# jczarnowski/DeepFactors

Hardware: NVIDIA H100
Metric: keyframe-pair Jacobian+JtJ evals/sec (640x480, C=32) (higher is better)
Workload: dtype f32

## Files before the change

### deepfactors_b200/_lib.py

```python
from __future__ import annotations

import ctypes as C
import os

_HERE = os.path.dirname(os.path.abspath(__file__))
LIB_PATH = os.environ.get("DFK_LIB") or os.path.join(_HERE, "libdfk.so")

DFK_OK = 0
DFK_ERR_INVALID_ARG = 1
DFK_ERR_CUDA = 2
DFK_ERR_UNSUPPORTED = 3
DFK_ERR_NOMEM = 4

DFK_GRAM_AUTO, DFK_GRAM_FP32, DFK_GRAM_TF32X3 = 0, 1, 2


class DfkError(RuntimeError):

    def __init__(self, status: int, message: str):
        super().__init__(f"dfk status {status}: {message}")
        self.status = status
        self.message = message


# ... 173 lines not shown


class DfkBowQuery(C.Structure):
    _fields_ = [("vector", DfkBowVector), ("max_results", C.c_int32), ("max_id", C.c_int32)]


class DfkBowScoreItem(C.Structure):
    _fields_ = [("entry", C.c_int32), ("vector", DfkBowVector)]


BOW_TRAIN_MAX_ROUNDS = 1000
BOW_TRAIN_MAX_DESCRIPTORS = 268435456


class DfkBowTrainDesc(C.Structure):
    _fields_ = [("k", C.c_int32), ("L", C.c_int32), ("descriptor_bytes", C.c_int32), ("num_images", C.c_int32),
                ("seed", C.c_uint64), ("num_descriptors", C.c_int64), ("descriptors_dev", C.c_void_p),
                ("image_offsets", C.c_void_p)]


class DfkBowTrainStats(C.Structure):
    _fields_ = [("num_nodes", C.c_int32), ("num_words", C.c_int32), ("max_rounds", C.c_int32),
                ("capped_nodes", C.c_int32), ("empty_clusters", C.c_int32),
                ("level_max_rounds", C.c_int32 * BOW_MAX_DEPTH)]


class DfkBowVocabularyShape(C.Structure):
    _fields_ = [("k", C.c_int32), ("L", C.c_int32), ("weighting", C.c_int32), ("scoring", C.c_int32),
                ("descriptor_bytes", C.c_int32), ("num_nodes", C.c_int32), ("num_words", C.c_int32)]


WINDOW_ERROR_DOUBLES = 7
WINDOW_ERROR_EX_DOUBLES = 8


_F = C.POINTER(C.c_float)
_IMG = C.POINTER(DfkImage)
_CAM = C.POINTER(DfkCamera)
_H = C.c_void_p
SYMBOLS = {
    "dfk_create": (C.c_int, [C.c_int, C.POINTER(_H)]),
    "dfk_destroy": (C.c_int, [_H]),
    "dfk_set_stream": (C.c_int, [_H, C.c_void_p]),
    "dfk_set_sm_limit": (C.c_int, [_H, C.c_int]),
    "dfk_use_own_stream": (C.c_int, [_H]),
    "dfk_get_stream": (C.c_void_p, [_H]),
    "dfk_synchronize": (C.c_int, [_H]),
    "dfk_last_error": (C.c_char_p, [_H]),
    "dfk_status_string": (C.c_char_p, [C.c_int]),
    "dfk_version": (C.c_int, []),
    "dfk_sfm_supports_code_size": (C.c_int, [C.c_int]),
    "dfk_set_profiling": (C.c_int, [_H, C.c_int]),
    "dfk_get_profile": (C.c_int, [_H, C.POINTER(C.c_double), C.POINTER(C.c_uint64), C.POINTER(C.c_uint64)]),
    "dfk_sfm_set_params": (C.c_int, [_H, C.POINTER(DfkSfmAlignerParams)]),
    "dfk_sfm_get_params": (C.c_int, [_H, C.POINTER(DfkSfmAlignerParams)]),
    "dfk_sfm_set_gram_mode": (C.c_int, [_H, C.c_int]),
    "dfk_se3_set_huber_delta": (C.c_int, [_H, C.c_float]),
    "dfk_sfm_run_step": (C.c_int, [_H, _F, _F, _F, C.c_int, _CAM, _IMG, _IMG, _IMG, _IMG, _IMG, _IMG, _IMG,
                                   _F, _F, _F, C.POINTER(C.c_uint64)]),
    "dfk_sfm_evaluate_error": (C.c_int, [_H, _F, _F, _CAM, _IMG, _IMG, _IMG, _IMG, _IMG, _F,
                                         C.POINTER(C.c_uint64)]),
    "dfk_sfm_evaluate_error_batch": (C.c_int, [_H, C.POINTER(DfkSfmWorkItem), C.c_int, C.c_void_p]),
    "dfk_sfm_run_step_batch": (C.c_int, [_H, C.POINTER(DfkSfmWorkItem), C.c_int, C.c_int, C.c_void_p]),
    "dfk_sfm_run_step_batch_host": (C.c_int, [_H, C.POINTER(DfkSfmWorkItem), C.c_int, C.c_int, _F]),
    "dfk_sfm_stream_create": (C.c_int, [_H, C.c_int, C.c_int, C.c_size_t, C.c_int, C.POINTER(C.c_void_p)]),
    "dfk_sfm_stream_destroy": (C.c_int, [_H, C.c_void_p]),
    "dfk_sfm_stream_submit": (C.c_int, [_H, C.c_void_p, C.POINTER(DfkSfmWorkItem), C.c_int, C.POINTER(C.c_uint64)]),
    "dfk_sfm_stream_wait": (C.c_int, [_H, C.c_void_p, C.c_uint64, _F]),
    "dfk_window_create": (C.c_int, [_H, C.POINTER(DfkWindowDesc), C.POINTER(C.c_void_p)]),
    "dfk_window_destroy": (C.c_int, [_H, C.c_void_p]),
    "dfk_window_floats": (C.c_size_t, [C.c_void_p]),
    "dfk_window_assemble": (C.c_int, [_H, C.c_void_p, C.c_void_p, C.c_void_p]),
    "dfk_window_create_geometric": (C.c_int, [_H, C.POINTER(DfkWindowDesc), C.c_int, C.POINTER(C.c_int32),
                                              C.POINTER(C.c_int32), C.POINTER(C.c_void_p)]),
    "dfk_window_assemble_geometric": (C.c_int, [_H, C.c_void_p, C.c_void_p, C.c_void_p, C.c_void_p]),
    "dfk_window_create_frames": (C.c_int, [_H, C.POINTER(DfkWindowDesc), C.c_int, C.POINTER(C.c_int32),
                                           C.POINTER(C.c_int32), C.c_int, C.POINTER(C.c_void_p)]),
    "dfk_window_marginalize_frames": (C.c_int, [_H, C.c_void_p, C.c_void_p, C.c_int, C.POINTER(C.c_int32), C.c_void_p,
                                                C.c_void_p]),
    "dfk_window_add_priors": (C.c_int, [_H, C.c_void_p, C.c_int, C.POINTER(C.c_int32), C.c_void_p, C.c_void_p,
                                        C.c_void_p]),
    "dfk_window_create_priors": (C.c_int, [_H, C.POINTER(DfkWindowDesc), C.c_int, C.POINTER(C.c_int32),
                                           C.POINTER(C.c_int32), C.c_int, C.c_int, C.POINTER(C.c_int32),
                                           C.POINTER(C.c_int32), C.POINTER(C.c_void_p)]),
    "dfk_window_add_keyframe_priors": (C.c_int, [_H, C.c_void_p, C.c_void_p, C.c_void_p, C.c_void_p]),
    "dfk_window_blanket": (C.c_int, [_H, C.c_void_p, C.c_int, C.POINTER(C.c_int32), C.POINTER(C.c_int32)]),
    "dfk_window_marginalize_keyframe": (C.c_int, [_H, C.c_void_p, C.c_void_p, C.c_void_p, C.c_int, C.c_int, C.c_void_p,
                                                  C.c_void_p, C.c_void_p, C.c_void_p, C.c_double,
                                                  C.POINTER(C.c_double), C.c_void_p, C.c_void_p]),
    "dfk_window_solver_create": (C.c_int, [_H, C.c_void_p, C.c_int, C.POINTER(C.c_int32), C.POINTER(C.c_void_p)]),
    "dfk_window_solver_destroy": (C.c_int, [_H, C.c_void_p]),
    "dfk_window_solver_tiles": (C.c_int, [_H, C.c_void_p, C.POINTER(C.c_size_t)]),
    "dfk_window_solve": (C.c_int, [_H, C.c_void_p, C.c_void_p, C.POINTER(DfkWindowSolveParams), C.POINTER(C.c_double),
                                   C.c_void_p, C.c_void_p]),
    "dfk_window_solver_update": (C.c_int, [_H, C.c_void_p, C.c_void_p, C.POINTER(DfkWindowUpdateParams),
                                           C.POINTER(C.c_double), C.c_void_p, C.c_void_p, C.POINTER(C.c_int32)]),
    "dfk_window_solver_create_from": (C.c_int, [_H, C.c_void_p, C.c_int, C.POINTER(C.c_int32), C.c_void_p,
                                                C.POINTER(C.c_void_p)]),
    "dfk_window_problem_create": (C.c_int, [_H, C.POINTER(DfkWindowProblemDesc), C.POINTER(C.c_void_p)]),
    "dfk_window_problem_destroy": (C.c_int, [_H, C.c_void_p]),
    "dfk_window_problem_set_state": (C.c_int, [_H, C.c_void_p, C.c_void_p, C.c_void_p]),
    "dfk_window_problem_get_state": (C.c_int, [_H, C.c_void_p, C.c_void_p, C.c_void_p]),
    "dfk_window_problem_linearize": (C.c_int, [_H, C.c_void_p, C.c_void_p]),
    "dfk_window_problem_error": (C.c_int, [_H, C.c_void_p, C.c_void_p]),
    "dfk_window_problem_retract": (C.c_int, [_H, C.c_void_p, C.c_void_p]),
    "dfk_window_problem_error_ex": (C.c_int, [_H, C.c_void_p, C.c_void_p]),
# ... 112 lines not shown
```

### deepfactors_b200/csrc/dfk_api.cu

```cuda
#include <cuda_runtime.h>
#include <math.h>
#include <stdint.h>
#include <stdio.h>
#include <stdlib.h>
#include <string.h>

#include <algorithm>
#include <cmath>
#include <memory>
#include <new>
#include <string>
#include <vector>

#include "dfk.h"
#include "dfk_host.h"
#include "dfk_internal.h"
#include "dfk_se3.cuh"

using namespace dfk;

struct DfkSfmStream {
  int device = 0, code_size = 0, max_items = 0, depth = 0;
  size_t max_bytes = 0;
  cudaStream_t copy_stream = nullptr;
// ... 259 lines not shown
namespace {

DfkStatus cache_ray_tables(DfkHandle h, SfmItemDev* items, int n)
{
  h->ray_pending.clear();
  if (h->ray_flush) {
    h->ray_cache.clear();
    h->ray_flush = false;
  }
  for (int i = 0; i < n; ++i) {
    SfmItemDev& d = items[i];
    const uint32_t W = d.width, H = d.height;
    size_t rt = 0;
    for (const auto& r : h->ray_cache) {
      if (r.fx == d.fx && r.fy == d.fy && r.u0 == d.u0 && r.v0 == d.v0 && r.w == W && r.h == H) break;
      ++rt;
    }
    if (rt == h->ray_cache.size()) {
      if (rt >= 256) h->ray_flush = true;
      DfkContext::RayTab r{d.fx, d.fy, d.u0, d.v0, W, H, {}, false};
      if (r.dev.ensure((size_t)W + H) != cudaSuccess)
        return fail(h, DFK_ERR_CUDA, "[SfmAligner::RunStep] scratch allocation failed");
      h->ray_cache.push_back(std::move(r));
    }
    d.ray_tab = h->ray_cache[rt].dev.ptr;
    if (!h->ray_cache[rt].built) h->ray_pending.push_back(rt);
  }
  return DFK_OK;
}

DfkStatus run_batch(DfkHandle h, const DfkSfmWorkItem* items, int n, int code_size, float* records_dev)
{
  if (!items || n <= 0 || !records_dev) return fail(h, DFK_ERR_INVALID_ARG, "[SfmAligner::RunStep] null/empty batch");
  StepKernel k;
  DFK_TRY(choose_step_kernel(h, items, n, code_size, &k));
  DeviceGuard guard(h->device);
  SfmLaunchPlan plan;
  bool any_fused = false;
  for (int i = 0; i < n; ++i) any_fused = any_fused || items[i].code != nullptr;
  if (any_fused)
    DFK_CUDA(h, h->codes_dev.ensure((size_t)n * code_size), "[SfmAligner::RunStep] scratch allocation failed");
  h->items_host.resize(n);
  DFK_TRY(build_items(h, items, n, code_size, k.tile_px, k.max_ctas, h->codes_dev.ptr, h->items_host.data(), &plan));
  DFK_TRY(cache_ray_tables(h, h->items_host.data(), n));
  if (any_fused) {
    h->codes_host.assign((size_t)n * code_size, 0.0f);
    for (int i = 0; i < n; ++i)
      if (items[i].code)
        memcpy(h->codes_host.data() + (size_t)i * code_size, items[i].code, sizeof(float) * code_size);
    DFK_CUDA(h, cudaMemcpyAsync(h->codes_dev.ptr, h->codes_host.data(), sizeof(float) * (size_t)n * code_size,
                                cudaMemcpyHostToDevice, h->stream),
             "[SfmAligner::RunStep] code upload failed");
  }
  DFK_CUDA(h, h->items_dev.ensure((size_t)n), "[SfmAligner::RunStep] scratch allocation failed");
  DFK_CUDA(h, h->partials_dev.ensure((size_t)plan.num_partials * k.pfloats), "[SfmAligner::RunStep] scratch allocation failed");
  SfmItemDev* items_dev = h->items_dev.ptr;
  DFK_CUDA(h, cudaMemcpyAsync(items_dev, h->items_host.data(), sizeof(SfmItemDev) * n, cudaMemcpyHostToDevice, h->stream),
           "[SfmAligner::RunStep] work list upload failed");
  if (!h->ray_pending.empty()) {
    DFK_CUDA(h, launch_sfm_ray_tables(items_dev, n, h->stream), "[SfmAligner::RunStep] kernel launch failed");
    for (size_t rt : h->ray_pending) h->ray_cache[rt].built = true;
    h->launches += 1;
  }
  return launch_step(h, k, code_size, items_dev, n, plan, h->partials_dev.ptr, records_dev);
}

}

extern "C" {

int dfk_version(void) { return DFK_VERSION; }

const char* dfk_status_string(DfkStatus s)
{
  switch (s) {
    case DFK_OK: return "ok";
    case DFK_ERR_INVALID_ARG: return "invalid argument";
    case DFK_ERR_CUDA: return "CUDA error";
    case DFK_ERR_UNSUPPORTED: return "unsupported";
    case DFK_ERR_NOMEM: return "out of memory";
  }
  return "unknown";
}

int dfk_sfm_supports_code_size(int code_size)
{
  return (sfm_fp32_supported(code_size) || sfm_wide_supported(code_size)) ? 1 : 0;
}

DfkStatus dfk_create(int device, DfkHandle* out)
{
  try {
    if (!out) return DFK_ERR_INVALID_ARG;
    *out = nullptr;
    int count = 0;
    cudaError_t e = cudaGetDeviceCount(&count);
    if (e != cudaSuccess || count == 0) return DFK_ERR_CUDA;
    if (device < 0) {
      if (cudaGetDevice(&device) != cudaSuccess) return DFK_ERR_CUDA;
    }
    if (device >= count) return DFK_ERR_INVALID_ARG;
    DfkContext* h = new (std::nothrow) DfkContext();
    if (!h) return DFK_ERR_NOMEM;
    h->device = device;
    h->params.sfmparams = DfkDenseSfmParams{0.1f, 1000.f, 2.0f, 0.0f, 2};
    h->params.step_threads = 32; h->params.step_blocks = 11; h->params.eval_threads = 224; h->params.eval_blocks = 66;
    DeviceGuard guard(device);
    bool ok = true;
    ok = ok && cudaDeviceGetAttribute(&h->num_sms, cudaDevAttrMultiProcessorCount, device) == cudaSuccess;
    ok = ok && cudaStreamCreateWithFlags(&h->own_stream, cudaStreamNonBlocking) == cudaSuccess;
    h->stream = h->own_stream;
// ... 31 lines not shown
  });
}

DfkStatus dfk_use_own_stream(DfkHandle h)
{
  return guarded(h, [&] {
    h->stream = h->own_stream;
    return DFK_OK;
  });
}

DfkStatus dfk_set_sm_limit(DfkHandle h, int num_sms)
{
  return guarded(h, [&] {
    if (num_sms < 0) return fail(h, DFK_ERR_INVALID_ARG, "[dfk_set_sm_limit] num_sms < 0");
    h->sm_limit = num_sms;
    return DFK_OK;
  });
}

void* dfk_get_stream(DfkHandle h) { return h ? h->stream : nullptr; }

DfkStatus dfk_synchronize(DfkHandle h)
{
  return guarded(h, [&] {
    DeviceGuard guard(h->device);
    DFK_CUDA(h, cudaStreamSynchronize(h->stream), "stream synchronize failed");
    return DFK_OK;
  });
}

const char* dfk_last_error(DfkHandle h) { return h ? h->err.c_str() : "null handle"; }

DfkStatus dfk_set_profiling(DfkHandle h, int enabled)
{
  return guarded(h, [&] {
    h->profiling = enabled != 0;
    return DFK_OK;
  });
}

DfkStatus dfk_get_profile(DfkHandle h, double* main_kernel_ms, uint64_t* main_kernel_launches,
                          uint64_t* total_kernel_launches)
{
  return guarded(h, [&] {
    DeviceGuard guard(h->device);
    DFK_TRY(drain_events(h));
    if (main_kernel_ms) *main_kernel_ms = h->ev_ms_accum;
    if (main_kernel_launches) *main_kernel_launches = h->ev_count_accum;
    if (total_kernel_launches) *total_kernel_launches = h->launches;
    h->ev_ms_accum = 0.0;
    h->ev_count_accum = 0;
    h->launches = 0;
    return DFK_OK;
  });
}

DfkStatus dfk_sfm_set_params(DfkHandle h, const DfkSfmAlignerParams* p)
{
  return guarded(h, [&] {
    if (!p) return DFK_ERR_INVALID_ARG;
    if (p->step_threads % 32 != 0 || p->eval_threads % 32 != 0)
      return fail(h, DFK_ERR_INVALID_ARG, "threads must be a multiple of 32!");
    if (p->step_blocks > 1024 || p->eval_blocks > 1024) return fail(h, DFK_ERR_INVALID_ARG, "blocks must be less than 1024");
    if (p->sfmparams.valid_border < 1)
      return fail(h, DFK_ERR_INVALID_ARG, "valid_border must be >= 1 (bilinear sampling reads ix+1, iy+1)");
    h->params = *p;
    return DFK_OK;
  });
}

DfkStatus dfk_sfm_get_params(DfkHandle h, DfkSfmAlignerParams* p)
{
  return guarded(h, [&] {
    if (!p) return DFK_ERR_INVALID_ARG;
    *p = h->params;
    return DFK_OK;
  });
}

DfkStatus dfk_sfm_set_gram_mode(DfkHandle h, DfkGramMode m)
{
  return guarded(h, [&] {
    if (m != DFK_GRAM_AUTO && m != DFK_GRAM_FP32 && m != DFK_GRAM_TF32X3)
      return fail(h, DFK_ERR_INVALID_ARG, "unknown gram mode");
    h->gram_mode = m;
    return DFK_OK;
  });
}

DfkStatus dfk_se3_set_huber_delta(DfkHandle h, float v)
{
  return guarded(h, [&] {
    h->se3_huber_delta = v;
    return DFK_OK;
  });
}

DfkStatus dfk_sfm_run_step_batch(DfkHandle h, const DfkSfmWorkItem* items, int n, int code_size, float* records_dev)
{
  return guarded(h, [&] { return run_batch(h, items, n, code_size, records_dev); });
}

DfkStatus dfk_sfm_run_step_batch_host(DfkHandle h, const DfkSfmWorkItem* items, int n, int code_size,
                                      float* records_host)
{
// ... 853 lines not shown
```

### deepfactors_b200/csrc/dfk_host.h

```cpp
#pragma once

#include <cuda_runtime.h>
#include <stdint.h>
#include <string.h>

#include <algorithm>
#include <string>
#include <vector>

#include "dfk.h"
#include "dfk_internal.h"
#include "dfk_se3.cuh"

using namespace dfk;

template <typename T, bool Pinned>
struct Scratch {
  T* ptr = nullptr;
  size_t cap = 0;

  Scratch() = default;
  Scratch(Scratch&& o) noexcept : ptr(o.ptr), cap(o.cap) { o.ptr = nullptr; o.cap = 0; }
  ~Scratch() { release(); }

// ... 35 lines not shown

  DeviceBuf<float> simple_scratch;
  DeviceBuf<unsigned int> counter;
  DeviceBuf<float> out_dev;
  PinnedBuf<float> out_host;
  DeviceBuf<float> code_dev;
  std::vector<unsigned char> staging;
  DeviceBuf<unsigned char> batch_dev;
  PinnedBuf<unsigned char> batch_host;
  DeviceBuf<float> batch_partials;
  DeviceBuf<unsigned int> batch_counters;
  DeviceBuf<unsigned char> eval_descs;
  DeviceBuf<float> eval_partials;
  DeviceBuf<unsigned int> eval_counters;
  DeviceBuf<unsigned char> depth_dev;
  DeviceBuf<unsigned char> depth_prior_dev;
  DeviceBuf<float> depth_prior_partials;

  DeviceBuf<unsigned char> sparse_dev;
  PinnedBuf<unsigned char> sparse_host;
  DeviceBuf<unsigned char> rep_dev;
  DeviceBuf<unsigned char> geo_dev;
  DeviceBuf<SfmItemDev> items_dev;
  DeviceBuf<float> partials_dev;
  DeviceBuf<unsigned char> match_items;
  DeviceBuf<unsigned char> match_scratch;
  DeviceBuf<unsigned char> orb_items;
  DeviceBuf<unsigned char> orb_scratch;
  DeviceBuf<unsigned char> orb_pyr_dev;
  DeviceBuf<unsigned char> pp_dev;
  DeviceBuf<double> pp_partials;
  DeviceBuf<unsigned char> mesh_dev;
  DeviceBuf<unsigned char> mesh_scratch;
  DeviceBuf<unsigned char> bow_dev;
  DeviceBuf<int32_t> bow_words;
  DeviceBuf<unsigned char> bow_scratch;
  DeviceBuf<int> window_lists;
  DeviceBuf<unsigned char> marg_lists;
  DeviceBuf<unsigned char> marg_dev;
  struct RayTab {
    float fx, fy, u0, v0;
    uint32_t w, h;
    DeviceBuf<float> dev;
    bool built;
  };
  std::vector<RayTab> ray_cache;
  std::vector<size_t> ray_pending;
  bool ray_flush = false;
  DeviceBuf<float> codes_dev;
  std::vector<float> codes_host;
  DeviceBuf<float> records_dev;
  PinnedBuf<float> records_host;
  std::vector<SfmItemDev> items_host;

  bool profiling = false;
  std::vector<cudaEvent_t> ev_pool;
  size_t ev_used = 0;
  double ev_ms_accum = 0.0;
  uint64_t ev_count_accum = 0;
  uint64_t launches = 0;

  ~DfkContext()
  {
    for (cudaEvent_t e : ev_pool) cudaEventDestroy(e);
    if (own_stream) cudaStreamDestroy(own_stream);
  }
};

inline DfkStatus fail(DfkHandle h, DfkStatus s, const std::string& msg)
{
  if (h) h->err = msg;
  return s;
}

inline DfkStatus oom(DfkHandle h) noexcept
{
  if (h) {
    try {
      h->err = "out of host memory";
    } catch (...) {
    }
  }
  return DFK_ERR_NOMEM;
}

template <class F>
DfkStatus guarded(DfkHandle h, F&& body) noexcept
{
  if (!h) return DFK_ERR_INVALID_ARG;
  try {
    return body();
  } catch (...) {
    return oom(h);
  }
}

inline DfkStatus cuda_fail(DfkHandle h, cudaError_t e, const char* what)
{
  std::string m = std::string(what) + ": " + cudaGetErrorString(e);
  cudaGetLastError();
  return fail(h, DFK_ERR_CUDA, m);
}

#define DFK_CUDA(h, call, what)                            \
  do {                                                     \
    cudaError_t e__ = (call);                              \
// ... 305 lines not shown
```

### deepfactors_b200/csrc/dfk_internal.h

```cpp
#pragma once

#include <cuda_runtime.h>
#include <stdint.h>

#include <string>
#include <vector>

#include "dfk.h"
#include "dfk_preprocess_model.h"

namespace dfk {

template <class T>
struct Part {
  size_t off = 0;
  T* at(void* base) const { return reinterpret_cast<T*>(static_cast<unsigned char*>(base) + off); }
};

struct Layout {
  size_t bytes = 0;
  template <class T>
  Part<T> add(size_t count)
  {
    const Part<T> p{bytes};
// ... 22 lines not shown
  uint32_t num_pixels;
  uint32_t tile_begin;
  uint32_t num_tiles;
  uint32_t perm_mul;
  uint32_t mag_tiles;
  uint32_t mag_width;
  uint32_t first_cta, num_ctas, partial_begin;
  uint32_t flags;
  float* dpt_out;
  uint32_t dpt_out_pitch;
  const float* code;
  const float* ray_tab;
  float P0[36];
  float P1[36];
};

enum : uint32_t { ITEM_FLAG_BULK = 1u, ITEM_FLAG_GRAD_ALIGNED = 2u, ITEM_FLAG_FUSED_DEPTH = 4u };

template <int C>
struct SfmCfg {
  static constexpr int NF = C + 7;
  static constexpr int NFP = (NF + 7) & ~7;
  static constexpr int NB = NFP / 8;
  static constexpr int NBLK = NB * (NB + 1) / 2;
  static constexpr int PARTIAL_FLOATS = NFP * NFP + 8;
};

constexpr int kTilePixels = 256;

template <int C>
struct TcCfg {
  static constexpr int S = C - 8;
  static constexpr int F = C + 8;
  static constexpr int ROWS = 2 * C;
  static constexpr int COLS = C + 24;
  static constexpr int PARTIAL_FLOATS = ROWS * COLS + 8;
  static constexpr int INLIERS = ROWS * COLS;
  __host__ __device__ static constexpr int hh(int i, int j) { return j * ROWS + S + i; }
  __host__ __device__ static constexpr int lh(int i, int j) { return i < S ? j * ROWS + i : (16 + i) * ROWS + S + j; }
};

constexpr int kSfmTcTilePixels = 128;
constexpr int sfm_tc_ctas_per_sm(int code_size) { return code_size <= 32 ? 4 : (code_size <= 64 ? 2 : 1); }
__host__ __device__ constexpr bool sfm_tc_writes_d(int code_size) { return code_size > 32; }
constexpr size_t sfm_tc_partial_floats(int code_size) { return (size_t)(2 * code_size) * (code_size + 24) + 8; }

struct SfmLaunchPlan {
  int num_items = 0;
  int num_tiles = 0;
  int num_ctas = 0;
  int num_partials = 0;
};

cudaError_t launch_sfm_fp32(int code_size, const SfmItemDev* items_dev, const SfmLaunchPlan& plan,
                            float* partials_dev, cudaStream_t stream, cudaEvent_t ev_start = nullptr,
                            cudaEvent_t ev_stop = nullptr);
cudaError_t launch_sfm_ray_tables(const SfmItemDev* items_dev, int num_items, cudaStream_t stream);
cudaError_t launch_sfm_finalize(int code_size, bool tc, const SfmItemDev* items_dev, int num_items,
                                const float* partials_dev, float* records_dev, cudaStream_t stream);
constexpr int sfm_wide_tile_pixels(int code_size) { return code_size >= 128 ? 64 : 128; }
bool sfm_wide_supported(int code_size);
cudaError_t launch_sfm_wide(int code_size, const SfmItemDev* items_dev, const SfmLaunchPlan& plan,
                            float* partials_dev, cudaStream_t stream, cudaEvent_t ev_start = nullptr,
                            cudaEvent_t ev_stop = nullptr);
bool sfm_tc_supported(int code_size);
cudaError_t launch_sfm_tc(int code_size, const SfmItemDev* items_dev, const SfmLaunchPlan& plan, float* partials_dev,
                          cudaStream_t stream, cudaEvent_t ev_start = nullptr, cudaEvent_t ev_stop = nullptr);
size_t sfm_partial_floats(int code_size);
constexpr int sfm_fp32_ctas_per_sm(int code_size) { return code_size <= 8 ? 2 : 1; }
bool sfm_fp32_supported(int code_size);
int sfm_max_ctas();

struct PixelCam {
  float q[4], t[3];
  float fx, fy, u0, v0, border, ulim, vlim, min_dpt;
};
struct View {
  const float* ptr;
  uint32_t pitch;
};
int grid_for(int area);
struct Se3TrackDesc {
  PixelCam pc;
  View img0, img1, dpt0, grad1;
  int width, height;
  int nblocks;
  int grad_aligned;
};
cudaError_t launch_se3_step(const Se3TrackDesc& d, float huber_delta, float* scratch, unsigned int* counter, float* out,
                            float* pose, float* history, cudaStream_t s);
cudaError_t launch_se3_step(const Se3TrackDesc* descs_dev, int num_problems, int max_blocks, float huber_delta,
                            float* scratch, int scratch_stride, unsigned int* counters, float* outs, float* poses,
                            cudaStream_t s);
struct EvalErrorDesc {
  PixelCam pc;
  View img0, img1, dpt0;
  int width, height;
  int nblocks;
  int scratch_row;
};
cudaError_t launch_eval_error(const EvalErrorDesc& d, float huber_delta, float* scratch, unsigned int* counter,
                              float* out, cudaStream_t s);
cudaError_t launch_eval_error(const EvalErrorDesc* descs_dev, int num_items, int max_blocks, float huber_delta,
                              float* scratch, unsigned int* counters, float* outs, cudaStream_t s);
struct DepthDecodeDesc {
  View prx, jac;
// ... 450 lines not shown
```

### deepfactors_b200/csrc/dfk_sfm_finalize.cu

```cuda
#include <cuda_runtime.h>
#include <stdint.h>

#include "dfk_internal.h"

namespace dfk {

namespace {

constexpr int kFinWarps = 8;
constexpr int kFinUnroll = 4;

__device__ __forceinline__ int packed_index(int i, int j, int NP) { return i * NP - (i * (i - 1)) / 2 + (j - i); }

template <int C, bool TC>
__global__ void __launch_bounds__(kFinWarps * 32)
sfm_finalize_kernel(const SfmItemDev* __restrict__ items, const float* __restrict__ partials,
                    float* __restrict__ records)
{
  using Cfg = SfmCfg<C>;
  constexpr int NFP = Cfg::NFP;
  constexpr int NP = 12 + C;
  constexpr int NH = NP * (NP + 1) / 2;
  constexpr int REC = NH + NP + 2;
  constexpr int NE = (C + 7 > 49) ? (C + 7) : 49;
  constexpr int EPL = (NE + 31) / 32;
  using Tc = TcCfg<C>;
  constexpr int PSTRIDE = TC ? Tc::PARTIAL_FLOATS : Cfg::PARTIAL_FLOATS;
  constexpr int INL_OFF = TC ? Tc::INLIERS : NFP * NFP;
  constexpr int NOFF = TC ? 3 : 1;
  __shared__ float red[kFinWarps][EPL * 32];
  __shared__ unsigned int red_inl[kFinWarps];
  __shared__ float sum[EPL * 32];

  cudaGridDependencySynchronize();
  const SfmItemDev& I = items[blockIdx.x];
  const int unit = blockIdx.y;
  const int warp = threadIdx.x >> 5, lane = threadIdx.x & 31;
  const float* P = partials + (size_t)I.partial_begin * PSTRIDE;
  const int np = (int)I.num_ctas;

  int off[EPL][NOFF];
  bool act[EPL];
#pragma unroll
  for (int q = 0; q < EPL; ++q) {
    const int e = q * 32 + lane;
    int fi, fj;
    if (unit < C) {
      act[q] = (unit + e) < (C + 7);
      fi = unit;
      fj = unit + e;
    } else {
      const int r = e / 7, c = e - 7 * r;
      act[q] = (e < 49) && (c >= r);
      fi = C + r;
      fj = C + c;
    }
    if (!act[q]) {
      fi = 0;
      fj = 0;
    }
    if constexpr (TC) {
      off[q][0] = Tc::hh(fi, fj);
      off[q][1] = Tc::lh(fi, fj);
      off[q][2] = Tc::lh(fj, fi);
    } else {
      off[q][0] = fi * NFP + fj;
    }
  }
  float part[EPL];
#pragma unroll
  for (int q = 0; q < EPL; ++q) part[q] = 0.0f;
  unsigned int inl = 0;
  for (int k0 = warp; k0 < np; k0 += kFinWarps * kFinUnroll) {
    float v[kFinUnroll][EPL];
    unsigned int vi[kFinUnroll];
#pragma unroll
    for (int u = 0; u < kFinUnroll; ++u) {
      const int k = k0 + u * kFinWarps;
      const bool on = k < np;
      const float* Pk = P + (size_t)(on ? k : 0) * PSTRIDE;
#pragma unroll
      for (int q = 0; q < EPL; ++q) {
        v[u][q] = 0.0f;
        if (on && act[q]) {
          if constexpr (TC) v[u][q] = (Pk[off[q][0]] + Pk[off[q][1]]) + Pk[off[q][2]];
          else v[u][q] = Pk[off[q][0]];
        }
// ... 127 lines not shown
```

### deepfactors_b200/csrc/dfk_sfm_tc.cu

```cuda
#include <cuda_runtime.h>
#include <stdint.h>

#include "dfk_async.cuh"
#include "dfk_geom.cuh"
#include "dfk_internal.h"
#include "dfk_sfm_frontend.cuh"
#include "dfk_wgmma.cuh"

namespace dfk {

namespace {

constexpr int TILE = kSfmTcTilePixels;
constexpr uint32_t kLbo = 128 + 16;
constexpr uint32_t kSbo = 32 * kLbo + 16;
#ifndef DFK_FLUSH_TILES
#define DFK_FLUSH_TILES 8
#endif
constexpr int kFlushTiles = DFK_FLUSH_TILES;

template <int C>
struct WgCfg {
  using T = TcCfg<C>;
  static constexpr int NWG = C >= 128 ? 2 : 1;
// ... 280 lines not shown
    if constexpr (W::NWG > 1) __syncthreads();
#pragma unroll
    for (int i4 = 0; i4 < NQ; ++i4) {
      if (i4 >= PRE) load_quad(i4);
      const float sk = __shfl_sync(0xffffffffu, feat[0], 4 * i4 + r);
#pragma unroll
      for (int cb = 0; cb < NCB; ++cb) {
        const float x[4] = {sk * v[i4][cb].x, sk * v[i4][cb].y, sk * v[i4][cb].z, sk * v[i4][cb].w};
        const uint32_t gh = code_h + (uint32_t)(4 * cb) * kSbo;
        const uint32_t gl = cb < NCB - 1 ? code_l + (uint32_t)(4 * cb) * kSbo : code_l_last;
#pragma unroll
        for (int e = 0; e < 4; ++e) {
          const float h = tf32_trunc(x[e]);
          const uint32_t off = (uint32_t)i4 * kLbo + (uint32_t)e * 16u;
          sts32(gh + off, h);
          sts32(gl + off, x[e] - h);
        }
      }
    }
    if (lane < PW) {
#pragma unroll
      for (int f = 0; f < 7; ++f) {
        const float h = tf32_trunc(feat[1 + f]);
        sts32(pose_h + (uint32_t)f * 16u, h);
        sts32(pose_l + (uint32_t)f * 16u, feat[1 + f] - h);
      }
    }
    fence_proxy_async_smem();
    const int nv = __syncthreads_count(ok);
    if (nv > 0) {
      wgmma_fence();
#pragma unroll
      for (int kk = 0; kk < TILE / 8; ++kk) {
        const uint32_t k_off = (uint32_t)kk * 2u * kLbo;
        const bool accumulate = kk > 0 || chain_valid > 0;
#ifndef DFK_EXP_NOMMA
        const uint64_t b_desc = make_wgmma_desc_kmajor(op + (uint32_t)W::G_H * kSbo + k_off, kLbo, kSbo);
#pragma unroll
        for (int t = 0; t < MT; ++t)
          wgmma_tf32<N>(acc[t], make_wgmma_desc_kmajor(op + (uint32_t)(8 * (MT * wg + t)) * kSbo + k_off, kLbo, kSbo),
                        b_desc, accumulate);
#endif
      }
      wgmma_commit();
    }
    chain_valid += nv;
    inliers += (unsigned)nv;
    ++tiles_in_chain;
#ifdef DFK_EXP_CTA_CLOCKS
    valid_tiles += nv > 0;
#endif
  }
  flush(true);
#ifdef DFK_EXP_CTA_CLOCKS
  __syncthreads();
  if (tid == 0 && blockIdx.x < kClockCtas) {
    unsigned int smid;
    asm volatile("mov.u32 %0, %%smid;" : "=r"(smid));
    unsigned long long* o = g_cta_clocks[blockIdx.x];
    o[0] = t_entry;
    o[1] = global_ns();
    o[2] = ((unsigned long long)ntiles << 32) | (unsigned)valid_tiles;
    o[3] = smid;
  }
#endif
}

template <int C>
cudaError_t launch_impl(const SfmItemDev* items_dev, const SfmLaunchPlan& plan, float* partials_dev,
                        cudaStream_t stream, cudaEvent_t ev_start, cudaEvent_t ev_stop)
{
  constexpr size_t smem = sizeof(Smem<C>);
  if constexpr (smem > 48 * 1024) {
    const cudaError_t err =
        cudaFuncSetAttribute(sfm_step_tc_kernel<C>, cudaFuncAttributeMaxDynamicSharedMemorySize, (int)smem);
    if (err != cudaSuccess) return err;
  }
  if (ev_start) cudaEventRecord(ev_start, stream);
  sfm_step_tc_kernel<C><<<plan.num_ctas, WgCfg<C>::THREADS, smem, stream>>>(items_dev, plan.num_tiles, partials_dev);
  if (ev_stop) cudaEventRecord(ev_stop, stream);
  return cudaGetLastError();
}

}

bool sfm_tc_supported(int code_size) { return code_size == 32 || code_size == 64 || code_size == 128; }

cudaError_t launch_sfm_tc(int code_size, const SfmItemDev* items_dev, const SfmLaunchPlan& plan, float* partials_dev,
                          cudaStream_t stream, cudaEvent_t ev_start, cudaEvent_t ev_stop)
{
  switch (code_size) {
    case 32: return launch_impl<32>(items_dev, plan, partials_dev, stream, ev_start, ev_stop);
    case 64: return launch_impl<64>(items_dev, plan, partials_dev, stream, ev_start, ev_stop);
    case 128: return launch_impl<128>(items_dev, plan, partials_dev, stream, ev_start, ev_stop);
    default: return cudaErrorInvalidValue;
  }
}

}

#ifdef DFK_EXP_CTA_CLOCKS
extern "C" int dfk_exp_cta_clocks(unsigned long long* out, int n)
{
  if (n < 0 || n > dfk::kClockCtas) return -1;
  if (cudaDeviceSynchronize() != cudaSuccess) return -1;
  return cudaMemcpyFromSymbol(out, dfk::g_cta_clocks, sizeof(unsigned long long) * 4 * (size_t)n) == cudaSuccess ? 0 : -1;
// ... 3 lines not shown
```

### deepfactors_b200/csrc/dfk_window.cu

```cuda
#include <cuda_runtime.h>
#include <stdint.h>

#include "dfk_internal.h"

namespace dfk {

namespace {

__device__ __forceinline__ int packed_index(int i, int j, int NP) { return i * NP - (i * (i - 1)) / 2 + (j - i); }
__device__ __forceinline__ float rec_h(const float* rec, int a, int b, int NP)
{
  return a <= b ? rec[packed_index(a, b, NP)] : rec[packed_index(b, a, NP)];
}

__device__ __forceinline__ int link_row0(int r) { return r < 6 ? r : 6 + r; }
__device__ __forceinline__ int link_row1(int r, int C) { return r < 6 ? 6 + r : 6 + C + r; }

__global__ void __launch_bounds__(256)
window_assemble_kernel(WindowDev w, const float* __restrict__ records, const float* __restrict__ geo,
                       float* __restrict__ out)
{
  const int C = w.code_size, B = 6 + C, NP = 12 + C;
  const int NH = NP * (NP + 1) / 2, REC = NH + NP + 2;
  const int NG = 12 + 2 * C, NHG = NG * (NG + 1) / 2, RECG = NHG + NG + 2;
  float* tail = out + (size_t)w.num_keyframes * (B * B + B) + (size_t)w.num_pairs * B * 6;
  const int job = blockIdx.x;
  if (job < w.num_keyframes) {
    const int k = job;
    float* D = out + (size_t)k * B * B;
    float* g = out + (size_t)w.num_keyframes * B * B + (size_t)k * B;
    const int a0 = w.kf0_ptr[k], a1 = w.kf0_ptr[k + 1];
    const int b0 = w.kf1_ptr[k], b1 = w.kf1_ptr[k + 1];
    const int l00 = w.lk0_ptr[k], l01 = w.lk0_ptr[k + 1];
    const int l10 = w.lk1_ptr[k], l11 = w.lk1_ptr[k + 1];
    for (int e = threadIdx.x; e < B * B + B; e += blockDim.x) {
      float s = 0.0f;
      if (e < B * B) {
        const int r = e / B, c = e - r * B;
        const int lr = r < 6 ? r : 6 + r, lc = c < 6 ? c : 6 + c;
        for (int q = a0; q < a1; ++q) s += rec_h(records + (size_t)w.kf0_items[q] * REC, lr, lc, NP);
        if (r < 6 && c < 6)
          for (int q = b0; q < b1; ++q) s += rec_h(records + (size_t)w.kf1_items[q] * REC, 6 + r, 6 + c, NP);
        for (int q = l00; q < l01; ++q) s += rec_h(geo + (size_t)w.lk0_links[q] * RECG, link_row0(r), link_row0(c), NG);
        for (int q = l10; q < l11; ++q)
          s += rec_h(geo + (size_t)w.lk1_links[q] * RECG, link_row1(r, C), link_row1(c, C), NG);
        D[e] = s;
      } else {
        const int r = e - B * B;
        const int lr = r < 6 ? r : 6 + r;
        for (int q = a0; q < a1; ++q) s -= records[(size_t)w.kf0_items[q] * REC + NH + lr];
        if (r < 6)
          for (int q = b0; q < b1; ++q) s -= records[(size_t)w.kf1_items[q] * REC + NH + 6 + r];
        for (int q = l00; q < l01; ++q) s -= geo[(size_t)w.lk0_links[q] * RECG + NHG + link_row0(r)];
        for (int q = l10; q < l11; ++q) s -= geo[(size_t)w.lk1_links[q] * RECG + NHG + link_row1(r, C)];
        g[r] = s;
      }
    }
  } else if (job < w.num_keyframes + w.num_pairs) {
    const int p = job - w.num_keyframes;
    float* O = out + (size_t)w.num_keyframes * (B * B + B) + (size_t)p * B * 6;
    const int i0 = w.pair_ptr[p], i1 = w.pair_ptr[p + 1];
    for (int e = threadIdx.x; e < B * 6; e += blockDim.x) {
      const int r = e / 6, c = e - r * 6;
      const int lr = r < 6 ? r : 6 + r;
      float s = 0.0f;
      for (int q = i0; q < i1; ++q) s += rec_h(records + (size_t)w.pair_items[q] * REC, lr, 6 + c, NP);
      O[e] = s;
    }
  } else if (job < w.num_keyframes + w.num_pairs + w.num_links) {
    const int l = job - w.num_keyframes - w.num_pairs;
    float* O = tail + 2 + (size_t)l * B * B;
    const float* rec = geo + (size_t)l * RECG;
    for (int e = threadIdx.x; e < B * B; e += blockDim.x) {
      const int r = e / B, c = e - r * B;
      O[e] = rec_h(rec, link_row0(r), link_row1(c, C), NG);
    }
  } else if (job < w.num_keyframes + w.num_pairs + w.num_links + w.num_frames) {
    const int f = job - w.num_keyframes - w.num_pairs - w.num_links;
    float* Df = tail + 2 + (size_t)w.num_links * B * B + (size_t)f * 36;
    float* gf = tail + 2 + (size_t)w.num_links * B * B + (size_t)w.num_frames * 36 + (size_t)f * 6;
    const int p = w.frame_pair[f];
    const int i0 = w.pair_ptr[p], i1 = w.pair_ptr[p + 1];
    for (int e = threadIdx.x; e < 42; e += blockDim.x) {
      float s = 0.0f;
      if (e < 36) {
        const int r = e / 6, c = e - r * 6;
        for (int q = i0; q < i1; ++q) s += rec_h(records + (size_t)w.pair_items[q] * REC, 6 + r, 6 + c, NP);
        Df[e] = s;
// ... 394 lines not shown
      for (int r = threadIdx.x; r < nB; r += blockDim.x) {
        double Gd = 0.0;
        for (int c = 0; c < nB; ++c) Gd = __fma_rn(P[(size_t)r * nB + c], d[c], Gd);
        gd = __fma_rn(P[(size_t)nB * nB + r], d[r], gd);
        dGd = __fma_rn(d[r], Gd, dGd);
      }
      gd = block_sum(gd, red);
      dGd = block_sum(dGd, red);
      f = __dadd_rn(f, __dadd_rn(__fma_rn(-2.0, gd, P[(size_t)nB * nB + nB]), dGd));
    }
  }
  if (threadIdx.x == 0) {
    if (md.w > 0.0) {
      double cc = 0.0;
      for (int c = 0; c < C; ++c) cc = __fma_rn(md.code[c], md.code[c], cc);
      f = __fma_rn(md.w, cc, f);
    }
    *md.f = f;
    *md.info = 0;
  }
}

__global__ void __launch_bounds__(256)
window_marg_finalize_kernel(int C, KfMargDev md, int num_tiles, double* __restrict__ prior)
{
  const int B = 6 + C, n = md.n, nB = n * B;
  const bool bad = *md.info != 0;
  const int u = blockIdx.x, nt = n * (n + 1) / 2;
  if (u < nt) {
    const int t = n + 1 + u, I = md.tile_row[t], J = md.tile_col[t];
    const double* T = md.tiles + (size_t)t * B * B;
    for (int e = threadIdx.x; e < B * B; e += blockDim.x) {
      const int r = e / B, c = e - r * B;
      if (I == J && r < c) continue;
      const double v = bad ? 0.0 : T[e];
      prior[(size_t)((I - 1) * B + r) * nB + (J - 1) * B + c] = v;
      prior[(size_t)((J - 1) * B + c) * nB + (I - 1) * B + r] = v;
    }
    return;
  }
  for (int v = threadIdx.x; v < nB; v += blockDim.x) prior[(size_t)nB * nB + v] = bad ? 0.0 : md.rhs[B + v];
  if (threadIdx.x == 0) {
    double zz = 0.0;
    for (int r = 0; r < B; ++r) zz = __fma_rn(md.rhs[r], md.rhs[r], zz);
    prior[(size_t)nB * nB + nB] = bad ? 0.0 : __dsub_rn(*md.f, zz);
  }
}

}

cudaError_t launch_window_assemble(const WindowDev& w, const float* records_dev, const float* geo_records_dev,
                                   float* out_dev, cudaStream_t stream)
{
  window_assemble_kernel<<<w.num_keyframes + w.num_pairs + w.num_links + w.num_frames + 1, 256, 0, stream>>>(
      w, records_dev, geo_records_dev, out_dev);
  return cudaGetLastError();
}

cudaError_t launch_window_marginalize_frames(const WindowDev& w, const float* records_dev, int n, const int* frames_dev,
                                             double* priors_dev, int32_t* info_dev, cudaStream_t stream)
{
  window_marginalize_kernel<<<n, 256, 0, stream>>>(w, records_dev, frames_dev, priors_dev, info_dev);
  return cudaGetLastError();
}

cudaError_t launch_window_add_priors(const WindowDev& w, int m, const int* kf_ptr_dev, const int* kf_priors_dev,
                                     const double* priors_dev, const double* delta_dev, float* window_dev,
                                     cudaStream_t stream)
{
  window_add_priors_kernel<<<w.num_keyframes + 1, 256, 0, stream>>>(w, m, kf_ptr_dev, kf_priors_dev, priors_dev,
                                                                    delta_dev, window_dev);
  return cudaGetLastError();
}

cudaError_t launch_window_add_keyframe_priors(const WindowDev& w, const KfPriorDev& kp, const double* priors_dev,
                                              const double* delta_dev, float* window_dev, cudaStream_t stream)
{
  window_add_kf_priors_kernel<<<w.num_keyframes + kp.num_blocks + 1, 256, 0, stream>>>(w, kp, priors_dev, delta_dev,
                                                                                       window_dev);
  return cudaGetLastError();
}

cudaError_t launch_window_marg_gather(const WindowDev& w, const KfPriorDev& kp, const KfMargDev& md, int num_tiles,
                                      cudaStream_t stream)
{
  window_marg_gather_kernel<<<num_tiles + 1, 256, 0, stream>>>(w, kp, md, num_tiles);
  return cudaGetLastError();
}

cudaError_t launch_window_marg_finalize(int code_size, const KfMargDev& md, int num_tiles, double* prior_dev,
                                       cudaStream_t stream)
{
  window_marg_finalize_kernel<<<md.n * (md.n + 1) / 2 + 1, 256, 0, stream>>>(code_size, md, num_tiles, prior_dev);
  return cudaGetLastError();
}

}
```

### include/dfk.h

```cpp
#ifndef DFK_H_
#define DFK_H_

#include <stddef.h>
#include <stdint.h>

#ifdef __cplusplus
extern "C" {
#endif

#define DFK_VERSION 104

typedef enum {
  DFK_OK = 0,
  DFK_ERR_INVALID_ARG = 1,
  DFK_ERR_CUDA = 2,
  DFK_ERR_UNSUPPORTED = 3,
  DFK_ERR_NOMEM = 4
} DfkStatus;

typedef struct DfkContext* DfkHandle;

typedef struct {
  void* ptr;
  size_t pitch_bytes;
  uint32_t width;
  uint32_t height;
} DfkImage;

typedef struct {
  float fx, fy, u0, v0;
  float width, height;
} DfkCamera;

typedef struct {
  float huber_delta;
  float ocl_th;
  float avg_dpt;
  float min_dpt;
  int32_t valid_border;
} DfkDenseSfmParams;

typedef struct {
  DfkDenseSfmParams sfmparams;
  int32_t step_threads;
  int32_t step_blocks;
  int32_t eval_threads;
  int32_t eval_blocks;
} DfkSfmAlignerParams;

typedef enum { DFK_GRAM_AUTO = 0, DFK_GRAM_FP32 = 1, DFK_GRAM_TF32X3 = 2 } DfkGramMode;


DfkStatus dfk_create(int device, DfkHandle* out);
DfkStatus dfk_destroy(DfkHandle h);
DfkStatus dfk_set_stream(DfkHandle h, void* cuda_stream);
DfkStatus dfk_use_own_stream(DfkHandle h);
DfkStatus dfk_set_sm_limit(DfkHandle h, int num_sms);
void* dfk_get_stream(DfkHandle h);
DfkStatus dfk_synchronize(DfkHandle h);
const char* dfk_last_error(DfkHandle h);
const char* dfk_status_string(DfkStatus s);
int dfk_version(void);
int dfk_sfm_supports_code_size(int code_size);

DfkStatus dfk_set_profiling(DfkHandle h, int enabled);
DfkStatus dfk_get_profile(DfkHandle h, double* main_kernel_ms, uint64_t* main_kernel_launches,
                          uint64_t* total_kernel_launches);

DfkStatus dfk_sfm_set_params(DfkHandle h, const DfkSfmAlignerParams* p);
DfkStatus dfk_sfm_get_params(DfkHandle h, DfkSfmAlignerParams* p);
DfkStatus dfk_sfm_set_gram_mode(DfkHandle h, DfkGramMode m);
DfkStatus dfk_se3_set_huber_delta(DfkHandle h, float v);


DfkStatus dfk_sfm_run_step(DfkHandle h, const float pose0[7], const float pose1[7],
                           const float* code0, int code_size, const DfkCamera* cam,
                           const DfkImage* img0, const DfkImage* img1, const DfkImage* dpt0,
                           const DfkImage* std0, const DfkImage* valid0, const DfkImage* prx0_jac,
                           const DfkImage* grad1,
                           float* JtJ, float* Jtr, float* residual, uint64_t* inliers);

DfkStatus dfk_sfm_evaluate_error(DfkHandle h, const float pose0[7], const float pose1[7],
                                 const DfkCamera* cam, const DfkImage* img0, const DfkImage* img1,
                                 const DfkImage* dpt0, const DfkImage* std0, const DfkImage* grad1,
                                 float* residual, uint64_t* inliers);

typedef struct {
  float pose0[7];
  float pose1[7];
  DfkCamera cam;
  DfkImage img0, img1, dpt0, valid0, prx0_jac, grad1;
  DfkImage prx_orig;
  const float* code;
} DfkSfmWorkItem;

#define DFK_SFM_NP(C) (12 + (C))
#define DFK_SFM_RECORD_FLOATS(C) (DFK_SFM_NP(C) * (DFK_SFM_NP(C) + 1) / 2 + DFK_SFM_NP(C) + 2)

DfkStatus dfk_sfm_run_step_batch(DfkHandle h, const DfkSfmWorkItem* items, int n, int code_size,
                                 float* records_dev);
DfkStatus dfk_sfm_run_step_batch_host(DfkHandle h, const DfkSfmWorkItem* items, int n, int code_size,
                                      float* records_host);

DfkStatus dfk_sfm_evaluate_error_batch(DfkHandle h, const DfkSfmWorkItem* items, int n, float* out_dev);

typedef struct DfkSfmStream DfkSfmStream;
DfkStatus dfk_sfm_stream_create(DfkHandle h, int code_size, int max_items, size_t max_bytes_per_submit, int depth,
                                DfkSfmStream** out);
DfkStatus dfk_sfm_stream_destroy(DfkHandle h, DfkSfmStream* s);
DfkStatus dfk_sfm_stream_submit(DfkHandle h, DfkSfmStream* s, const DfkSfmWorkItem* host_items, int n,
                                uint64_t* ticket);
DfkStatus dfk_sfm_stream_wait(DfkHandle h, DfkSfmStream* s, uint64_t ticket, float* records_host);

typedef struct DfkWindow DfkWindow;
typedef struct {
  int32_t num_keyframes;
  int32_t num_pairs;
  int32_t num_items;
  int32_t code_size;
  const int32_t* pair_k0;
// ... 450 lines not shown
```

Before: 33530.

## Skip redundant work-list uploads, chain step kernels with PDL, split window assembly

Caches the last uploaded SfM work list on the host and skips the host-to-device copy when it matches byte-for-byte on the same stream. It also adds programmatic launch-completion triggers to the step and finalize kernels and launches window assembly with programmatic stream serialization, so dependent kernels can start their prologue early. The keyframe assembly job is split across several blocks per keyframe instead of one block striding over all elements. The memcmp costs host time every call, and reusing device contents assumes nothing else overwrote the items buffer.

```diff
diff --git a/deepfactors_b200/_lib.py b/deepfactors_b200/_lib.py
--- a/deepfactors_b200/_lib.py
+++ b/deepfactors_b200/_lib.py
@@ -249,6 +249,7 @@
     "dfk_sfm_supports_code_size": (C.c_int, [C.c_int]),
     "dfk_set_profiling": (C.c_int, [_H, C.c_int]),
     "dfk_get_profile": (C.c_int, [_H, C.POINTER(C.c_double), C.POINTER(C.c_uint64), C.POINTER(C.c_uint64)]),
+    "dfk_get_work_list_uploads": (C.c_int, [_H, C.POINTER(C.c_uint64)]),
     "dfk_sfm_set_params": (C.c_int, [_H, C.POINTER(DfkSfmAlignerParams)]),
     "dfk_sfm_get_params": (C.c_int, [_H, C.POINTER(DfkSfmAlignerParams)]),
     "dfk_sfm_set_gram_mode": (C.c_int, [_H, C.c_int]),
diff --git a/deepfactors_b200/csrc/dfk_api.cu b/deepfactors_b200/csrc/dfk_api.cu
--- a/deepfactors_b200/csrc/dfk_api.cu
+++ b/deepfactors_b200/csrc/dfk_api.cu
@@ -335,11 +335,20 @@
                                 cudaMemcpyHostToDevice, h->stream),
              "[SfmAligner::RunStep] code upload failed");
   }
+  if (h->items_dev.cap < (size_t)n) h->items_kept.clear();
   DFK_CUDA(h, h->items_dev.ensure((size_t)n), "[SfmAligner::RunStep] scratch allocation failed");
   DFK_CUDA(h, h->partials_dev.ensure((size_t)plan.num_partials * k.pfloats), "[SfmAligner::RunStep] scratch allocation failed");
   SfmItemDev* items_dev = h->items_dev.ptr;
-  DFK_CUDA(h, cudaMemcpyAsync(items_dev, h->items_host.data(), sizeof(SfmItemDev) * n, cudaMemcpyHostToDevice, h->stream),
-           "[SfmAligner::RunStep] work list upload failed");
+  const bool same = h->items_kept.size() == (size_t)n && h->items_kept_stream == h->stream &&
+                    memcmp(h->items_kept.data(), h->items_host.data(), sizeof(SfmItemDev) * n) == 0;
+  if (!same) {
+    h->items_kept.clear();
+    DFK_CUDA(h, cudaMemcpyAsync(items_dev, h->items_host.data(), sizeof(SfmItemDev) * n, cudaMemcpyHostToDevice, h->stream),
+             "[SfmAligner::RunStep] work list upload failed");
+    h->items_kept.assign(h->items_host.begin(), h->items_host.end());
+    h->items_kept_stream = h->stream;
+    h->work_list_uploads += 1;
+  }
   if (!h->ray_pending.empty()) {
     DFK_CUDA(h, launch_sfm_ray_tables(items_dev, n, h->stream), "[SfmAligner::RunStep] kernel launch failed");
     for (size_t rt : h->ray_pending) h->ray_cache[rt].built = true;
@@ -477,6 +486,15 @@
     h->ev_ms_accum = 0.0;
     h->ev_count_accum = 0;
     h->launches = 0;
+    return DFK_OK;
+  });
+}
+
+DfkStatus dfk_get_work_list_uploads(DfkHandle h, uint64_t* uploads)
+{
+  return guarded(h, [&] {
+    if (!uploads) return fail(h, DFK_ERR_INVALID_ARG, "[dfk_get_work_list_uploads] null argument");
+    *uploads = h->work_list_uploads;
     return DFK_OK;
   });
 }
diff --git a/deepfactors_b200/csrc/dfk_host.h b/deepfactors_b200/csrc/dfk_host.h
--- a/deepfactors_b200/csrc/dfk_host.h
+++ b/deepfactors_b200/csrc/dfk_host.h
@@ -111,6 +111,9 @@
   DeviceBuf<float> records_dev;
   PinnedBuf<float> records_host;
   std::vector<SfmItemDev> items_host;
+  std::vector<SfmItemDev> items_kept;
+  cudaStream_t items_kept_stream = nullptr;
+  uint64_t work_list_uploads = 0;
 
   bool profiling = false;
   std::vector<cudaEvent_t> ev_pool;
diff --git a/deepfactors_b200/csrc/dfk_internal.h b/deepfactors_b200/csrc/dfk_internal.h
--- a/deepfactors_b200/csrc/dfk_internal.h
+++ b/deepfactors_b200/csrc/dfk_internal.h
@@ -98,6 +98,12 @@
   int num_partials = 0;
 };
 
+#ifdef DFK_UNCHAINED_STEP
+constexpr bool kChainStep = false;
+#else
+constexpr bool kChainStep = true;
+#endif
+
 cudaError_t launch_sfm_fp32(int code_size, const SfmItemDev* items_dev, const SfmLaunchPlan& plan,
                             float* partials_dev, cudaStream_t stream, cudaEvent_t ev_start = nullptr,
                             cudaEvent_t ev_stop = nullptr);
diff --git a/deepfactors_b200/csrc/dfk_sfm_finalize.cu b/deepfactors_b200/csrc/dfk_sfm_finalize.cu
--- a/deepfactors_b200/csrc/dfk_sfm_finalize.cu
+++ b/deepfactors_b200/csrc/dfk_sfm_finalize.cu
@@ -33,6 +33,7 @@
   __shared__ float sum[EPL * 32];
 
   cudaGridDependencySynchronize();
+  if constexpr (kChainStep) cudaTriggerProgrammaticLaunchCompletion();
   const SfmItemDev& I = items[blockIdx.x];
   const int unit = blockIdx.y;
   const int warp = threadIdx.x >> 5, lane = threadIdx.x & 31;
diff --git a/deepfactors_b200/csrc/dfk_sfm_tc.cu b/deepfactors_b200/csrc/dfk_sfm_tc.cu
--- a/deepfactors_b200/csrc/dfk_sfm_tc.cu
+++ b/deepfactors_b200/csrc/dfk_sfm_tc.cu
@@ -356,6 +356,7 @@
 #endif
   }
   flush(true);
+  if constexpr (kChainStep) cudaTriggerProgrammaticLaunchCompletion();
 #ifdef DFK_EXP_CTA_CLOCKS
   __syncthreads();
   if (tid == 0 && blockIdx.x < kClockCtas) {
diff --git a/deepfactors_b200/csrc/dfk_window.cu b/deepfactors_b200/csrc/dfk_window.cu
--- a/deepfactors_b200/csrc/dfk_window.cu
+++ b/deepfactors_b200/csrc/dfk_window.cu
@@ -16,7 +16,13 @@
 __device__ __forceinline__ int link_row0(int r) { return r < 6 ? r : 6 + r; }
 __device__ __forceinline__ int link_row1(int r, int C) { return r < 6 ? 6 + r : 6 + C + r; }
 
-__global__ void __launch_bounds__(256)
+constexpr int kAssembleThreads = 256;
+__host__ __device__ constexpr int assemble_keyframe_blocks(int C)
+{
+  return ((6 + C) * (6 + C) + (6 + C) + kAssembleThreads - 1) / kAssembleThreads;
+}
+
+__global__ void __launch_bounds__(kAssembleThreads)
 window_assemble_kernel(WindowDev w, const float* __restrict__ records, const float* __restrict__ geo,
                        float* __restrict__ out)
 {
@@ -24,7 +30,9 @@
   const int NH = NP * (NP + 1) / 2, REC = NH + NP + 2;
   const int NG = 12 + 2 * C, NHG = NG * (NG + 1) / 2, RECG = NHG + NG + 2;
   float* tail = out + (size_t)w.num_keyframes * (B * B + B) + (size_t)w.num_pairs * B * 6;
-  const int job = blockIdx.x;
+  cudaGridDependencySynchronize();
+  const int S = assemble_keyframe_blocks(C), kf_blocks = w.num_keyframes * S;
+  const int job = (int)blockIdx.x < kf_blocks ? (int)blockIdx.x / S : (int)blockIdx.x - kf_blocks + w.num_keyframes;
   if (job < w.num_keyframes) {
     const int k = job;
     float* D = out + (size_t)k * B * B;
@@ -33,7 +41,8 @@
     const int b0 = w.kf1_ptr[k], b1 = w.kf1_ptr[k + 1];
     const int l00 = w.lk0_ptr[k], l01 = w.lk0_ptr[k + 1];
     const int l10 = w.lk1_ptr[k], l11 = w.lk1_ptr[k + 1];
-    for (int e = threadIdx.x; e < B * B + B; e += blockDim.x) {
+    const int e = ((int)blockIdx.x - k * S) * kAssembleThreads + (int)threadIdx.x;
+    if (e < B * B + B) {
       float s = 0.0f;
       if (e < B * B) {
         const int r = e / B, c = e - r * B;
@@ -534,9 +543,17 @@
 cudaError_t launch_window_assemble(const WindowDev& w, const float* records_dev, const float* geo_records_dev,
                                    float* out_dev, cudaStream_t stream)
 {
-  window_assemble_kernel<<<w.num_keyframes + w.num_pairs + w.num_links + w.num_frames + 1, 256, 0, stream>>>(
-      w, records_dev, geo_records_dev, out_dev);
-  return cudaGetLastError();
+  cudaLaunchConfig_t cfg{};
+  cfg.gridDim = dim3(w.num_keyframes * assemble_keyframe_blocks(w.code_size) + w.num_pairs + w.num_links + w.num_frames + 1);
+  cfg.blockDim = dim3(kAssembleThreads);
+  cfg.dynamicSmemBytes = 0;
+  cfg.stream = stream;
+  cudaLaunchAttribute attr[1];
+  attr[0].id = cudaLaunchAttributeProgrammaticStreamSerialization;
+  attr[0].val.programmaticStreamSerializationAllowed = 1;
+  cfg.attrs = attr;
+  cfg.numAttrs = kChainStep ? 1 : 0;
+  return cudaLaunchKernelEx(&cfg, window_assemble_kernel, w, records_dev, geo_records_dev, out_dev);
 }
 
 cudaError_t launch_window_marginalize_frames(const WindowDev& w, const float* records_dev, int n, const int* frames_dev,
diff --git a/include/dfk.h b/include/dfk.h
--- a/include/dfk.h
+++ b/include/dfk.h
@@ -66,6 +66,7 @@
 DfkStatus dfk_set_profiling(DfkHandle h, int enabled);
 DfkStatus dfk_get_profile(DfkHandle h, double* main_kernel_ms, uint64_t* main_kernel_launches,
                           uint64_t* total_kernel_launches);
+DfkStatus dfk_get_work_list_uploads(DfkHandle h, uint64_t* uploads);
 
 DfkStatus dfk_sfm_set_params(DfkHandle h, const DfkSfmAlignerParams* p);
 DfkStatus dfk_sfm_get_params(DfkHandle h, DfkSfmAlignerParams* p);
```

Result: faster. 34480 (median of 6 runs) (+2.9%).
